# 1879615351/Go-RIO

Hardware: AMD Instinct MI355X
Metric: APD-GICP GN iters/sec on 16k-pt scans + GP-preint windows/sec (higher is better)
Workload: dtype f32 search / f64 accumulate; 1 GPU; C4: 64 scan pairs 16384x16384 + 64 GP windows 1 s @ 200 Hz per GPU, k-NN covariances + 20 fixed GN iterations per pair; pairs_per_gpu=64, target_points=16384, optimizer=GN (convergence test disabled), search=pruned, parallelism=batch shard x1 (no collective)

## Files before the change

go-rio_amd/csrc/ugpm_api.hip:

```cpp
#include <hip/hip_runtime.h>

#include <algorithm>
#include <cstdlib>
#include <chrono>
#include <cstdio>
#include <cstring>
#include <limits>
#include <memory>
#include <string>
#include <atomic>
#include <vector>

#include "../../include/gorio_ugpm.h"
#include "dev_buffer.h"
#include "ugpm_kernels.hip"
#include "ugpm_lpm_out.hip"
#include "ugpm_chunks.h"
#include "ugpm_windows.h"

using namespace gorio;
using namespace gorio::windows;

namespace {

// ... 334 lines not shown
  if (which == 2) {
    if (npad <= 256) ug::ata_kernel<4, 16, kAtaTilesCorr><<<grid, 512, lds(16), sq>>>(r.wins, which, r.nw, ng, decide, dense);
    else if (npad <= 512) ug::ata_kernel<8, 16, kAtaTilesCorr><<<grid, 512, lds(16), sq>>>(r.wins, which, r.nw, ng, decide, dense);
    else ug::ata_kernel<16, 8, kAtaTilesCorr><<<grid, 512, lds(8), sq>>>(r.wins, which, r.nw, ng, decide, dense);
  } else {
    if (npad <= 256) ug::ata_kernel<4, 16, kAtaTilesLm><<<grid, 512, lds(16), sq>>>(r.wins, which, r.nw, ng, decide, dense);
    else ug::ata_kernel<8, 16, kAtaTilesLm><<<grid, 512, lds(16), sq>>>(r.wins, which, r.nw, ng, decide, dense);
  }
}

int enqueue_tables_and_correlation(Ctx& c, Batch& b) {
  const int max_S = b.max_S;
  for (const Run& r : b.runs) {
    {
      Stage st(c, 0, r.s);
      ug::lpm_rot_kernel<<<dim3(r.nw, 5), 320, 0, r.s>>>(r.wins);
      ug::lpm_init_kernel<<<r.nw, 320, 0, r.s>>>(r.wins);
    }
    {
      Stage st(c, 1, r.s);
      ug::gram_kernel<<<dim3(6, r.nw), 256, 0, r.s>>>(r.wins);
      ug::cross_kernel<<<dim3(12, r.nw, (std::max(b.max_G, b.max_V) + ug::kCrossRows - 1) / ug::kCrossRows), 256, sizeof(double) * ug::kCrossRows * (((max_S + 31) / 32) * 32 + 4), r.s>>>(r.wins);
    }
    UHIP(hipEventRecord(r.ev_tab, r.s));
    UHIP(hipStreamWaitEvent(r.s2, r.ev_tab, 0));
    {
      Stage st(c, 2, r.s2);
      ug::corr_jac_kernel<<<dim3(ug::kCorrJacParts, r.nw), 256, 0, r.s2>>>(r.wins);
      UHIP(hipEventRecord(r.ev_jac, r.s2));
      launch_ata(c, max_S, r, 2);
      ug::corr_factor_kernel<<<r.nw, 512, 0, r.s2>>>(r.wins);
// ... 82 lines not shown
    const Run& r = b.runs[g];
    if (problem == 0) {
      UHIP(hipStreamWaitEvent(r.s, r.ev_jac, 0));
      ug::lm_turn_kernel<<<r.nw, 256, 0, r.s>>>(r.wins, c.d_diag + 4 * (size_t)r.g0);
    }
    st_lm[g].reset();
  }
  return 0;
}

int enqueue_finish_and_infer(Ctx& c, Batch& b) {
  for (const Run& r : b.runs) {
    UHIP(hipStreamWaitEvent(r.s, r.ev_corr, 0));
    {
      Stage st(c, 4, r.s);
      ug::finish_kernel<<<r.nw, 256, 0, r.s>>>(r.wins, c.d_diag + 4 * (size_t)r.g0);
      ug::infer_kernel<<<dim3(std::max(1, b.max_infer), r.nw), 256, sizeof(double) * 17 * (6 * b.max_S + 16), r.s>>>(r.wins);
    }
    UHIP(hipEventRecord(r.ev_done, r.s));
  }
  for (size_t g = 1; g < b.runs.size(); ++g) UHIP(hipStreamWaitEvent(c.main.s, b.runs[g].ev_done, 0));
  UHIP(hipGetLastError());
  return 0;
}

int collect(Ctx& c, Batch& b, gorio_ugpm_meas* out, gorio_ugpm_diag* diag, std::vector<int>& unfinished) {
  double* const rec = static_cast<double*>(c.pin_out.get());
  double* const dg = rec + b.total_out;
  int* const fin = reinterpret_cast<int*>(dg + 4 * (size_t)b.nw);
  UHIP(hipMemcpyAsync(fin, c.d_ints, sizeof(int) * kWinInts * (size_t)b.nw, hipMemcpyDeviceToHost, c.main.s));
  UHIP(hipMemcpyAsync(dg, c.d_diag, sizeof(double) * 4 * (size_t)b.nw, hipMemcpyDeviceToHost, c.main.s));
// ... 119 lines not shown
  w->min_freq = 500;
  w->quantum = -1;
  w->state_freq = 50.0;
  w->correlate = 1;
  w->overlap = 8;
  w->vel_bias_std = 0.3;
  w->gyr_bias_std = 0.03;
}

const char* gorio_ugpm_last_error(void) { return g_err.c_str(); }

void gorio_ugpm_debug_set_schedule(int speculative_rot) { g_speculative_rot.store(speculative_rot ? 1 : 0); }

void gorio_ugpm_debug_set_path(int flags) { g_debug_path.store(flags); }

int gorio_ugpm_get_stage_times(double seconds[8], int counts[8]) {
  for (int i = 0; i < 8; ++i) {
    if (seconds) seconds[i] = g_stage_s[i];
    if (counts) counts[i] = g_stage_n[i];
  }
  return 0;
}

int gorio_ugpm_preint_batch(const gorio_ugpm_window* windows, int n_windows, gorio_ugpm_meas* out, gorio_ugpm_diag* diag, int device) {
  if (!windows || n_windows <= 0 || !out) return ufail(GORIO_UGPM_ERR_INVALID, "gorio_ugpm_preint_batch: bad arguments");
  bool any_chunked = false;
  for (int i = 0; i < n_windows; ++i) any_chunked = any_chunked || windows[i].quantum >= 0;
  if (!any_chunked) return preint_batch_flat(windows, n_windows, out, diag, device, false);
  struct Req { int first = 0, count = 0, status = 0; chunks::Plan plan; size_t out0 = 0; };
  std::vector<Req> reqs(n_windows);
// ... 105 lines not shown
```

go-rio_amd/csrc/ugpm_kernels.hip:

```cpp
#include <hip/hip_runtime.h>
#include <math.h>

#include "ugpm_device.h"

namespace gorio {
namespace ug {

__device__ __forceinline__ UgpmWin load_win(const UgpmWin* __restrict__ wins, int i) {
  UgpmWin w;
  __builtin_memcpy(&w, (const __attribute__((address_space(4))) void*)(wins + i), sizeof(UgpmWin));
  return w;
}


#ifndef GORIO_UGPM_XCD
#define GORIO_UGPM_XCD 1
#endif
struct WinPart {
  int win, part, z;
};
__device__ __forceinline__ WinPart xcd_win_part() {
  WinPart r{(int)blockIdx.y, (int)blockIdx.x, (int)blockIdx.z};
#if GORIO_UGPM_XCD
  if (gridDim.y >= 16u && (gridDim.y & 7u) == 0u) {
    const unsigned int inner = gridDim.x * gridDim.z;
    const unsigned int L = blockIdx.x + gridDim.x * (blockIdx.y + gridDim.y * blockIdx.z);
    const unsigned int slot = L >> 3, in = slot % inner;
    r.win = (int)((slot / inner) * 8u + (L & 7u));
    r.part = (int)(in % gridDim.x);
    r.z = (int)(in / gridDim.x);
  }
#endif
  return r;
}

constexpr double kDt = 0.01;
constexpr double kBw = 0.0001;
constexpr double kExpTol = 1e-14;
constexpr double kPi = 3.14159265358979323846;

struct V3 {
  double x, y, z;
};
struct M3 {
  double m[9];
};
__device__ __forceinline__ V3 v3(double x, double y, double z) { return V3{x, y, z}; }
__device__ __forceinline__ V3 operator+(V3 a, V3 b) { return V3{a.x + b.x, a.y + b.y, a.z + b.z}; }
__device__ __forceinline__ V3 operator-(V3 a, V3 b) { return V3{a.x - b.x, a.y - b.y, a.z - b.z}; }
__device__ __forceinline__ V3 operator*(double s, V3 a) { return V3{s * a.x, s * a.y, s * a.z}; }
__device__ __forceinline__ double vnorm(V3 a) { return sqrt(a.x * a.x + a.y * a.y + a.z * a.z); }
__device__ __forceinline__ V3 cross(V3 a, V3 b) { return V3{a.y * b.z - a.z * b.y, a.z * b.x - a.x * b.z, a.x * b.y - a.y * b.x}; }
__device__ __forceinline__ M3 eye3() { return M3{{1, 0, 0, 0, 1, 0, 0, 0, 1}}; }
__device__ __forceinline__ M3 mmul(const M3& a, const M3& b) {
// ... 222 lines not shown
    if (bl == 0) storeM(Rq + (size_t)idx * 9, R);
    else if (bl == 1) storeM(Rq + (size_t)(S + idx) * 9, R);
    else if (bl == 2) storeM(w.Rstart + variant * 9, R);
    else if (bl == 4 && variant == 0) {
      const V3 vr = mvec(R, v3(w.vel[idx] - w.vel_bias[0], w.vel[V + idx] - w.vel_bias[1], w.vel[2 * V + idx] - w.vel_bias[2]));
      w.velr[idx] = vr.x;
      w.velr[V + idx] = vr.y;
      w.velr[2 * V + idx] = vr.z;
    }
    interp(bt, w_prev);
    t_prev = bt;
  }
}

constexpr int kLpmMaxT = 2048;
struct LpmLds {
  double tl[kLpmMaxT];
  unsigned short kind[kLpmMaxT];
  unsigned short kidx[kLpmMaxT];
  double tot[2][256][9];
  double ps[9];
  int start_rank;
};

__device__ __forceinline__ int lower_bound_f(int n, double v, const double* __restrict__ a, double shift) {
  int lo = 0, hi = n;
  while (lo < hi) {
    const int mid = (lo + hi) >> 1;
    if (a[mid] - shift < v) lo = mid + 1; else hi = mid;
  }
  return lo;
}
__device__ __forceinline__ int upper_bound_f(int n, double v, const double* __restrict__ a, double shift) {
  int lo = 0, hi = n;
  while (lo < hi) {
    const int mid = (lo + hi) >> 1;
    if (a[mid] - shift <= v) lo = mid + 1; else hi = mid;
  }
  return lo;
}

__device__ bool lpm_rotation_parallel(const UgpmWin& w, int variant, LpmLds& L, double* __restrict__ Rseq , size_t rseq_cap) {
  const int S = w.S, G = w.G, V = w.V;
  const int nthr = blockDim.x, tid = threadIdx.x;
  const double lpm_start = w.state_t[0];
  const double tshift = variant == 1 ? kDt : 0.0;
  int nfake = 0;
  double fake_first = 0.0, fake_q = 0.0;
  {
    double first = w.state_t[0], top1 = -1e300, top2 = -1e300;
    auto consider = [&](double c) {
      if (c > top1) { top2 = top1; top1 = c; } else if (c > top2) { top2 = c; }
    };
    consider(w.state_t[S - 1]); if (S > 1) consider(w.state_t[S - 2]);
    consider(w.state_t[S - 1] + kDt); if (S > 1) consider(w.state_t[S - 2] + kDt);
    consider(w.start_t);
    consider(lpm_start + kDt); consider(lpm_start);
    consider(w.vel_t[V - 1] - tshift); if (V > 1) consider(w.vel_t[V - 2] - tshift);
    first = fmin(first, fmin(w.start_t, w.vel_t[0] - tshift));
    if ((top1 - top2) > (1.0 / 500.0)) {
      const int nb = (int)floor((top1 - first) * 500.0);
      if (nb > 0) { nfake = nb; fake_first = first; fake_q = (top1 - first) / ((double)nb); }
    }
  }
  const int T = 2 * S + 3 + V + nfake;
  if (T > kLpmMaxT || (size_t)T * 9 > rseq_cap) return false;
  auto count_in = [&](int l, double v, bool upper) -> int {
    switch (l) {
      case 0: return upper ? upper_bound_f(S, v, w.state_t, 0.0) : lower_bound_f(S, v, w.state_t, 0.0);
      case 1: return upper ? upper_bound_f(S, v, w.state_t, -kDt) : lower_bound_f(S, v, w.state_t, -kDt);
      case 2: return upper ? (w.start_t <= v ? 1 : 0) : (w.start_t < v ? 1 : 0);
      case 3: { const double a0 = lpm_start, a1 = lpm_start + kDt; return upper ? ((a0 <= v) + (a1 <= v)) : ((a0 < v) + (a1 < v)); }
      case 4: return upper ? upper_bound_f(V, v, w.vel_t, tshift) : lower_bound_f(V, v, w.vel_t, tshift);
      default: {
        int lo = 0, hi = nfake;
        while (lo < hi) {
          const int mid = (lo + hi) >> 1;
          const double c = fake_first + mid * fake_q;
          if (upper ? (c <= v) : (c < v)) lo = mid + 1; else hi = mid;
        }
        return lo;
      }
    }
  };
  const int prio[6] = {1, 2, 3, 0, 4, 5};
  const int nl[6] = {S, S, 1, 2, V, nfake};
  for (int e = tid; e < T; e += nthr) {
    int l = 0, i = e;
    while (i >= nl[l]) { i -= nl[l]; ++l; }
    double v;
    switch (l) {
      case 0: v = w.state_t[i]; break;
      case 1: v = w.state_t[i] + kDt; break;
      case 2: v = w.start_t; break;
      case 3: v = lpm_start + (i ? kDt : 0.0); break;
      case 4: v = w.vel_t[i] - tshift; break;
      default: v = fake_first + i * fake_q; break;
    }
    int rank = i;
    for (int b = 0; b < 6; ++b)
      if (b != l && nl[b] > 0) rank += count_in(b, v, prio[b] < prio[l]);
    L.tl[rank] = v;
    L.kind[rank] = (unsigned short)l;
    L.kidx[rank] = (unsigned short)i;
    if (l == 3 && i == 0) L.start_rank = rank;
  }
  __syncthreads();
  auto gt = [&](int i) -> double { return w.gyr_t[i] - tshift; };
  auto gd = [&](int a, int i) -> double {
    double d = w.gyr[a * G + i];
    if (variant == 0) d -= w.gyr_bias[a];
    if (variant - 2 == a) d += kBw;
    return d;
  };
  const double gt0 = gt(0);
  auto step_rot = [&](int i) -> M3 {
    const double t = L.tl[i];
    int p = 0;
    if (t > gt0) {
      p = lower_bound_f(G, t, w.gyr_t, tshift) - 1;
      if (p > G - 2) p = G - 2;
      if (p < 0) p = 0;
    }
    const double t0 = gt(p), t1 = gt(p + 1);
    double wv[3];
    for (int a = 0; a < 3; ++a) {
      const double d0 = gd(a, p), d1 = gd(a, p + 1);
      const double al = (d1 - d0) / (t1 - t0);
      const double be = d0 - (al * t0);
      wv[a] = al * t + be;
    }
    const double dt = L.tl[i + 1] - t;
    return expMap(v3(wv[0] * dt, wv[1] * dt, wv[2] * dt));
  };
  const int nch = nthr < 256 ? nthr : 256;
  const int ch = (T + nch - 1) / nch;
  if (tid < nch) {
    M3 acc = eye3();
    const int i0 = tid * ch, i1 = min(T, i0 + ch);
    for (int i = i0; i < i1; ++i) {
      storeM(Rseq + (size_t)i * 9, acc);
      if (i < T - 1) acc = mmul(acc, step_rot(i));
    }
    storeM(&L.tot[0][tid][0], acc);
  }
  __syncthreads();
  int cur = 0;
  for (int off = 1; off < nch; off <<= 1) {
    if (tid < nch) {
      M3 m = loadM(&L.tot[cur][tid][0]);
      if (tid >= off) m = mmul(loadM(&L.tot[cur][tid - off][0]), m);
      storeM(&L.tot[cur ^ 1][tid][0], m);
    }
    __syncthreads();
    cur ^= 1;
  }
  if (tid < nch) {
    const M3 pre = tid > 0 ? loadM(&L.tot[cur][tid - 1][0]) : eye3();
    const int i0 = tid * ch, i1 = min(T, i0 + ch);
    for (int i = i0; i < i1; ++i) {
      const M3 Pi = mmul(pre, loadM(Rseq + (size_t)i * 9));
      storeM(Rseq + (size_t)i * 9, Pi);
      if (i == L.start_rank) storeM(L.ps, mtr(Pi));
    }
  }
  __syncthreads();
  const M3 PsT = loadM(L.ps);
  double* Rq = w.Rq + (size_t)variant * 2 * S * 9;
  for (int i = tid; i < T; i += nthr) {
    const int l = L.kind[i], idx = L.kidx[i];
    if (l == 5 || l == 3) continue;
    if (l == 4 && variant != 0) continue;
    const M3 Pi = loadM(Rseq + (size_t)i * 9);
    const M3 R = i >= L.start_rank ? mmul(PsT, Pi) : Pi;
    if (l == 0) storeM(Rq + (size_t)idx * 9, R);
    else if (l == 1) storeM(Rq + (size_t)(S + idx) * 9, R);
    else if (l == 2) storeM(w.Rstart + variant * 9, R);
    else {
      const V3 vr = mvec(R, v3(w.vel[idx] - w.vel_bias[0], w.vel[V + idx] - w.vel_bias[1], w.vel[2 * V + idx] - w.vel_bias[2]));
      w.velr[idx] = vr.x;
      w.velr[V + idx] = vr.y;
      w.velr[2 * V + idx] = vr.z;
    }
  }
  __syncthreads();
  return true;
}

__device__ void lpm_position(const UgpmWin& w, int axis) {
  const int S = w.S, V = w.V;
  const double start = w.state_t[0];
  const double* vt = w.vel_t;
  const double* vd = w.velr + (size_t)axis * V;
  int data_ptr = 0;
  while (vt[data_ptr + 1] < start) {
    data_ptr++;
    if (data_ptr == V - 1) {
      *w.status = -3;
      return;
    }
// ... 60 lines not shown
          if (d < best) {
            best = d;
            id = q;
            bc = c;
          }
        }
        prev[j] = bc;
        rev[j] += (id - 1);
      }
      store3(r0 + (size_t)i * 3, prev[0]);
      store3(r1 + (size_t)i * 3, prev[1]);
    }
  }
}

__global__ __launch_bounds__(320) void lpm_rot_kernel(const UgpmWin* __restrict__ wins) {
  const UgpmWin w = load_win(wins, blockIdx.x);
  if (*w.status != 0) return;
  const int var = blockIdx.y, lane = threadIdx.x & 63;
  __shared__ LpmLds lds;
  {
    const size_t cap = ((size_t)(3 * w.S + 3 * w.G) * 3 * w.S) / 5;
    double* Rseq = w.Jrot + (size_t)var * cap;
    if (!lpm_rotation_parallel(w, var, lds, Rseq, cap)) {
      if (threadIdx.x == 0) lpm_rotation(w, var);
    }
  }
  __syncthreads();
  if (var == 0 && threadIdx.x < 3) lpm_position(w, threadIdx.x);
  if (threadIdx.x == 64) unwrap_variant(w, var);
  (void)lane;
}

__device__ void lm_begin_block(const UgpmWin& w, int problem);

__global__ __launch_bounds__(320) void lpm_init_kernel(const UgpmWin* __restrict__ wins) {
  const UgpmWin w = load_win(wins, blockIdx.x);
  if (*w.status != 0) return;
  const int S = w.S;
  const M3 sRt0 = mtr(loadM(w.Rstart));
  for (int i = threadIdx.x; i < S; i += blockDim.x) {
    const V3 a0 = load3(w.r0 + (size_t)i * 3), a1 = load3(w.r1 + (size_t)i * 3);
    const V3 d = (1.0 / kDt) * (a1 - a0);
    w.s_dr[i] = d.x; w.s_dr[S + i] = d.y; w.s_dr[2 * S + i] = d.z;
    const V3 vel = mvec(sRt0, (1.0 / kDt) * (load3(w.dp + ((size_t)S + i) * 3) - load3(w.dp + (size_t)i * 3)));
    w.s_vel[i] = vel.x; w.s_vel[S + i] = vel.y; w.s_vel[2 * S + i] = vel.z;
// ... 1427 lines not shown
  {
    const int rows = ((n + 15) / 16 - jb) * 16;
    for (int q = threadIdx.x; q < rows * 16; q += blockDim.x) Xc[(size_t)(q >> 4) * 17 + (q & 15)] = (q >> 4) == (q & 15) ? 1.0 : 0.0;
  }
  blocked_lower_solve16(w.Ac, n, jb, Xc, sh);
  if (threadIdx.x < 16) {
    const int c = threadIdx.x, col = j0 + c;
    const int rows = ((n + 15) / 16 - jb) * 16;
    double ssq = 0.0;
    for (int r = 0; r < rows; ++r) ssq = __builtin_fma(Xc[(size_t)r * 17 + c], Xc[(size_t)r * 17 + c], ssq);
    if (col < n) w.dsc[col] = w.sstd[col] * (1.0 / sqrt(ssq));
  }
}


__global__ __launch_bounds__(256) void finish_kernel(const UgpmWin* __restrict__ wins, double* __restrict__ diag_out ) {
  const UgpmWin w = load_win(wins, blockIdx.x);
  if (*w.status != 0) return;
  if (!lm_end_block(w, 1, diag_out + 4 * (size_t)blockIdx.x)) return;
  __syncthreads();
  const int S = w.S;
  for (int q = threadIdx.x; q < 6 * S; q += blockDim.x) {
    const int c = q / S, i = q % S;
    const double* s = c < 3 ? w.s_dr + (size_t)c * S : w.s_vel + (size_t)(c - 3) * S;
    w.alpha[q] = row_dot(w.Kinv + ((size_t)c * S + i) * S, s, S);
  }
  for (int q = threadIdx.x; q < 3 * S; q += blockDim.x) {
    const int a = q / S, i = q % S;
    w.state_r[q] = row_dot(w.KintKinv + ((size_t)a * S + i) * S, w.s_dr + (size_t)a * S, S) + (w.state_t[i] - w.start_t) * w.hyper[a * 4 + 3];
  }
  __syncthreads();
  for (int i = threadIdx.x; i < S; i += blockDim.x) {
    const V3 ri = v3(w.state_r[i], w.state_r[S + i], w.state_r[2 * S + i]);
    const M3 Ji = JrInv(ri);
    const V3 d_r = mvec(Ji, load3(w.d_r_dt_local + (size_t)i * 3));
// ... 32 lines not shown
      }
    const V3 sv = v3(w.s_vel[i], w.s_vel[S + i], w.s_vel[2 * S + i]) + mean_vel;
    const M3 dvbw = mmul(mmul(skew(sv), Jr(v3(-ri.x, -ri.y, -ri.z))), drbw);
    const V3 dvdt = (1.0 / kDt) * (mvec(dRt, sv) - sv);
    const double dv[3] = {dvdt.x, dvdt.y, dvdt.z};
    for (int a = 0; a < 3; ++a) {
      for (int c = 0; c < 3; ++c) {
        w.d_vel_bv[((size_t)a * S + i) * 3 + c] = R.m[a * 3 + c];
        w.d_vel_bw[((size_t)a * S + i) * 3 + c] = -dvbw.m[a * 3 + c];
      }
      w.d_vel_dt[a * S + i] = dv[a];
    }
  }
}

__global__ __launch_bounds__(256) void infer_kernel(const UgpmWin* __restrict__ wins) {
  const WinPart wp = xcd_win_part();
  const UgpmWin w = load_win(wins, wp.win);
  const int qi = wp.part;
  if (qi >= w.n_infer) return;
  double* out = w.out + (size_t)qi * 83;
  if (*w.status != 0) {
    for (int k = threadIdx.x; k < 83; k += blockDim.x) out[k] = __longlong_as_double(0x7ff8000000000000LL);
    return;
  }
  const int S = w.S, n = 6 * S;
  const double t = w.infer_t[qi], dt = t - w.start_t;
  __shared__ double ksv[6][160];
  __shared__ double ksd[3][160];
  __shared__ double ksK[6][160];
  __shared__ double sval[6][8];
  __shared__ double sval2[6][4];
  __shared__ double sred[8];
  __shared__ double scov[36];
  for (int q = threadIdx.x; q < 6 * S; q += blockDim.x) {
    const int c = q / S, j = q - c * S;
    ksv[c][j] = se_kint(w.start_t, t, w.state_t[j], w.hyper[c * 4], w.hyper[c * 4 + 1]);
    if (c >= 3) ksd[c - 3][j] = se_kint_dt(w.start_t, t, w.state_t[j], w.hyper[c * 4], w.hyper[c * 4 + 1]);
  }
  __syncthreads();
  for (int q = threadIdx.x; q < 6 * S; q += blockDim.x) {
    const int c = q / S, j = q - c * S;
    const double* Kc = w.Kinv + (size_t)c * S * S + j;
    double s = 0.0;
    for (int k = 0; k < S; ++k) s += ksv[c][k] * Kc[(size_t)k * S];
    ksK[c][j] = s;
  }
  __syncthreads();
  {
    const int wv = threadIdx.x >> 6, lane = threadIdx.x & 63;
    for (int c = wv; c < 6; c += (int)(blockDim.x >> 6)) {
      double acc[9] = {0, 0, 0, 0, 0, 0, 0, 0, 0};
      for (int j = lane; j < S; j += 64) {
        const double ks = ksv[c][j], kk = ksK[c][j];
        acc[0] += ks * w.alpha[c * S + j];
        acc[1] += kk * ks;
        if (c < 3) {
          acc[2] += kk * w.d_d_r_dt[c * S + j];
          for (int q = 0; q < 3; ++q) acc[3 + q] += kk * w.d_state_bw[((size_t)c * S + j) * 3 + q];
        } else {
          acc[2] += ksd[c - 3][j] * w.alpha[c * S + j] + kk * w.d_vel_dt[(c - 3) * S + j];
          for (int q = 0; q < 3; ++q) {
            acc[3 + q] += kk * w.d_vel_bw[((size_t)(c - 3) * S + j) * 3 + q];
// ... 8 lines not shown
      if (lane == 0) {
        const double l2 = w.hyper[c * 4], sf2 = w.hyper[c * 4 + 1];
        double var = kss_int(w.start_t, t, l2, sf2) - acc[1];
        if (var <= 0) var = dt * dt * w.hyper[c * 4 + 2];
        sval[c][0] = acc[0] + dt * w.hyper[c * 4 + 3];
        sval[c][1] = var;
        sval[c][2] = acc[2];
        for (int q = 0; q < 3; ++q) {
          sval[c][3 + q] = acc[3 + q];
          sval2[c][q] = acc[6 + q];
        }
      }
    }
  }
  __syncthreads();
  if (w.correlate) {
    extern __shared__ double Xc[];
    __shared__ Solve16Lds sh;
    const int rows = ((n + 15) / 16) * 16;
    for (int q = threadIdx.x; q < rows * 16; q += blockDim.x) Xc[(size_t)(q >> 4) * 17 + (q & 15)] = 0.0;
    __syncthreads();
    for (int row = threadIdx.x; row < n; row += blockDim.x) {
      const int c = row / S;
      Xc[(size_t)row * 17 + c] = w.dsc[row] * ksK[c][row - c * S];
    }
    blocked_lower_solve16(w.Ac, n, 0, Xc, sh);
    for (int pair = 0; pair < 21; ++pair) {
      int a2 = 0, b2 = pair;
      while (b2 >= 6 - a2) { b2 -= 6 - a2; ++a2; }
      b2 += a2;
      double acc = 0.0;
      for (int k = threadIdx.x; k < rows; k += blockDim.x) acc += Xc[(size_t)k * 17 + a2] * Xc[(size_t)k * 17 + b2];
      acc = block_sum(acc, sred);
      if (threadIdx.x == 0) {
        scov[a2 * 6 + b2] = acc;
        scov[b2 * 6 + a2] = acc;
      }
    }
  } else {
    if (threadIdx.x < 36) scov[threadIdx.x] = 0.0;
    __syncthreads();
    if (threadIdx.x < 6) {
      const int a2 = threadIdx.x;
      double s2 = 0.0;
      for (int j = 0; j < S; ++j) s2 += ksK[a2][j] * w.var[a2 * S + j] * ksK[a2][j];
      scov[a2 * 6 + a2] = s2;
    }
  }
  __syncthreads();
  if (threadIdx.x == 0) {
    const V3 r = v3(sval[0][0], sval[1][0], sval[2][0]);
    const M3 jr = Jr(r);
    const M3 R = expMap(r);
    M3 d_r_dw, d_p_dw, d_p_dv;
    for (int a = 0; a < 3; ++a)
      for (int q = 0; q < 3; ++q) {
        d_r_dw.m[a * 3 + q] = sval[a][3 + q];
        d_p_dw.m[a * 3 + q] = sval[3 + a][3 + q];
        d_p_dv.m[a * 3 + q] = sval2[3 + a][q];
      }
    storeM(out, R);
    out[9] = sval[3][0]; out[10] = sval[4][0]; out[11] = sval[5][0];
    out[12] = dt;
    out[13] = 0.5 * dt * dt;
// ... 28 lines not shown
      }
      for (int a = 0; a < 6; ++a)
        for (int b = 0; b < 6; ++b) {
          double s = 0.0;
          for (int k = 0; k < 6; ++k) s += J[a * 6 + k] * bc[k] * J[b * 6 + k];
          cov[a * 6 + b] += s;
        }
    }
    for (int q = 0; q < 36; ++q) out[14 + q] = cov[q];
    storeM(out + 50, mmul(jr, d_r_dw));
    store3(out + 59, mvec(jr, v3(sval[0][2], sval[1][2], sval[2][2])));
    storeM(out + 62, d_p_dw);
    storeM(out + 71, d_p_dv);
    out[80] = sval[3][2]; out[81] = sval[4][2]; out[82] = sval[5][2];
  }
}

}
}
```

go-rio_amd/ugpm.py:

```python
import ctypes as C

import numpy as np

from .apd import GorioError, load_library

LPM, UGPM = 0, 1
REC = 83

UGPM_SYMBOLS = ["gorio_ugpm_default_window", "gorio_ugpm_preint_batch", "gorio_ugpm_last_error", "gorio_ugpm_get_stage_times", "gorio_ugpm_debug_set_schedule",
                "gorio_ugpm_debug_set_path",                 "gorio_ugpm_combine_preints"]


class UgpmWindow(C.Structure):

    _fields_ = [
        ("gyr_t", C.c_void_p), ("gyr", C.c_void_p), ("n_gyr", C.c_int),
        ("vel_t", C.c_void_p), ("vel", C.c_void_p), ("n_vel", C.c_int),
        ("gyr_var", C.c_double), ("vel_var", C.c_double), ("start_t", C.c_double),
        ("infer_t", C.c_void_p), ("n_infer", C.c_int), ("type", C.c_int),
        ("min_freq", C.c_double), ("quantum", C.c_double), ("state_freq", C.c_double),
        ("correlate", C.c_int), ("overlap", C.c_int),
        ("gyr_bias", C.c_double * 3), ("vel_bias", C.c_double * 3),
        ("vel_bias_std", C.c_double), ("gyr_bias_std", C.c_double),
        ("group_sizes", C.c_void_p), ("n_groups", C.c_int),
# ... 98 lines not shown
    a, b, out = np.ascontiguousarray(pack(prev)), np.ascontiguousarray(pack(cur)), np.zeros(REC)
    lib.gorio_ugpm_combine_preints.argtypes = [C.c_void_p, C.c_void_p, C.c_void_p]
    rc = lib.gorio_ugpm_combine_preints(C.c_void_p(_dp(a)), C.c_void_p(_dp(b)), C.c_void_p(_dp(out)))
    if rc < 0:
        raise GorioError(rc, lib.gorio_ugpm_last_error().decode())
    return unpack(out)


def ugpm_debug_set_schedule(speculative_rot=True):
    lib = load_library()
    lib.gorio_ugpm_debug_set_schedule.argtypes = [C.c_int]
    lib.gorio_ugpm_debug_set_schedule.restype = None
    lib.gorio_ugpm_debug_set_schedule(1 if speculative_rot else 0)


def ugpm_debug_set_path(dense_ata=False, draining_looks=False):
    lib = load_library()
    lib.gorio_ugpm_debug_set_path.argtypes = [C.c_int]
    lib.gorio_ugpm_debug_set_path.restype = None
    lib.gorio_ugpm_debug_set_path((1 if dense_ata else 0) | (2 if draining_looks else 0))


def ugpm_stage_times():
    lib = load_library()
    s = (C.c_double * 8)()
    c = (C.c_int * 8)()
    lib.gorio_ugpm_get_stage_times(s, c)
    return list(s), list(c)


class PreintOption:

    def __init__(self, min_freq=500.0, type=UGPM, quantum=-1.0, state_freq=50.0, correlate=True):
        self.min_freq, self.type, self.quantum, self.state_freq, self.correlate = min_freq, type, quantum, state_freq, correlate

# ... 59 lines not shown
```

Baseline: 180,800 linearisations/s.

## Parallelise UGPM head/tail stages: staged LDS timestamps, parallel position/unwrap, tiled finish dots

Stages the state, velocity and gyro timestamp arrays into LDS for the LPM rotation kernel and packs the kind/index arrays into one word. The formerly single-thread position integration and unwrap tail are replaced by a parallel precompute of segment coefficients, query ranks and log maps, leaving only a short serial sweep. finish_kernel now computes its row dot products through LDS-tiled loads, and infer_kernel's 21 covariance reductions are fused into a single pass with wave shuffles. A debug flag keeps the old serial path, and optional cycle-counter instrumentation is added behind a compile macro.

```diff
diff --git a/go-rio_amd/csrc/ugpm_api.hip b/go-rio_amd/csrc/ugpm_api.hip
--- a/go-rio_amd/csrc/ugpm_api.hip
+++ b/go-rio_amd/csrc/ugpm_api.hip
@@ -372,7 +372,7 @@
   for (const Run& r : b.runs) {
     {
       Stage st(c, 0, r.s);
-      ug::lpm_rot_kernel<<<dim3(r.nw, 5), 320, 0, r.s>>>(r.wins);
+      ug::lpm_rot_kernel<<<dim3(r.nw, 5), 320, 0, r.s>>>(r.wins, (g_debug_path.load() & 4) ? 1 : 0);
       ug::lpm_init_kernel<<<r.nw, 320, 0, r.s>>>(r.wins);
     }
     {
@@ -485,7 +485,7 @@
     UHIP(hipStreamWaitEvent(r.s, r.ev_corr, 0));
     {
       Stage st(c, 4, r.s);
-      ug::finish_kernel<<<r.nw, 256, 0, r.s>>>(r.wins, c.d_diag + 4 * (size_t)r.g0);
+      ug::finish_kernel<<<r.nw, 256, 0, r.s>>>(r.wins, c.d_diag + 4 * (size_t)r.g0, (g_debug_path.load() & 4) ? 1 : 0);
       ug::infer_kernel<<<dim3(std::max(1, b.max_infer), r.nw), 256, sizeof(double) * 17 * (6 * b.max_S + 16), r.s>>>(r.wins);
     }
     UHIP(hipEventRecord(r.ev_done, r.s));
@@ -635,6 +635,15 @@
 
 void gorio_ugpm_debug_set_path(int flags) { g_debug_path.store(flags); }
 
+#ifdef GORIO_HT_TIMING
+int gorio_ugpm_debug_head_tail_cycles(long long cycles[32]) {
+  long long z[32] = {};
+  if (hipDeviceSynchronize() != hipSuccess) return -1;
+  if (cycles && hipMemcpyFromSymbol(cycles, HIP_SYMBOL(gorio::ug::g_ht_t), sizeof z) != hipSuccess) return -1;
+  return hipMemcpyToSymbol(HIP_SYMBOL(gorio::ug::g_ht_t), z, sizeof z) == hipSuccess ? 0 : -1;
+}
+#endif
+
 int gorio_ugpm_get_stage_times(double seconds[8], int counts[8]) {
   for (int i = 0; i < 8; ++i) {
     if (seconds) seconds[i] = g_stage_s[i];
diff --git a/go-rio_amd/csrc/ugpm_kernels.hip b/go-rio_amd/csrc/ugpm_kernels.hip
--- a/go-rio_amd/csrc/ugpm_kernels.hip
+++ b/go-rio_amd/csrc/ugpm_kernels.hip
@@ -38,6 +38,24 @@
 constexpr double kBw = 0.0001;
 constexpr double kExpTol = 1e-14;
 constexpr double kPi = 3.14159265358979323846;
+
+#ifdef GORIO_HT_TIMING
+__device__ long long g_ht_t[32];
+#define HT_T(k, thr)                                                                        \
+  do {                                                                                      \
+    if (blockIdx.x == 0 && blockIdx.y == 0 && (int)threadIdx.x == (thr)) {                  \
+      const long long now_ = (long long)__builtin_readcyclecounter();                       \
+      g_ht_t[k] += now_ - ht_last_;                                                         \
+      ht_last_ = now_;                                                                      \
+    }                                                                                       \
+  } while (0)
+#define HT_T_INIT long long ht_last_ = (long long)__builtin_readcyclecounter()
+#define HT_T_RESET ht_last_ = (long long)__builtin_readcyclecounter()
+#else
+#define HT_T(k, thr) do { } while (0)
+#define HT_T_INIT do { } while (0)
+#define HT_T_RESET do { } while (0)
+#endif
 
 struct V3 {
   double x, y, z;
@@ -290,14 +308,26 @@
 }
 
 constexpr int kLpmMaxT = 2048;
+constexpr int kLpmStage = 1000;
+constexpr int kLpmPos = 2 * 256 * 9;
 struct LpmLds {
-  double tl[kLpmMaxT];
-  unsigned short kind[kLpmMaxT];
-  unsigned short kidx[kLpmMaxT];
-  double tot[2][256][9];
+  union {
+    struct {
+      double tl[kLpmMaxT];
+      unsigned short kk[kLpmMaxT];
+    } line;
+    double uw[2 * 160 * 7];
+  };
+  union {
+    double tot[2][256][9];
+    double pos[kLpmPos];
+  };
+  double stage[kLpmStage];
   double ps[9];
   int start_rank;
+  int data_ptr;
 };
+static_assert(sizeof(LpmLds) <= 65536, "lpm_rot_kernel: static LDS");
 
 __device__ __forceinline__ int lower_bound_f(int n, double v, const double* __restrict__ a, double shift) {
   int lo = 0, hi = n;
@@ -316,24 +346,29 @@
   return lo;
 }
 
-__device__ bool lpm_rotation_parallel(const UgpmWin& w, int variant, LpmLds& L, double* __restrict__ Rseq , size_t rseq_cap) {
+template <bool STAGED>
+__device__ __forceinline__ bool lpm_rotation_parallel(const UgpmWin& w, int variant, LpmLds& L, double* __restrict__ Rseq , size_t rseq_cap) {
   const int S = w.S, G = w.G, V = w.V;
   const int nthr = blockDim.x, tid = threadIdx.x;
-  const double lpm_start = w.state_t[0];
+  const double* __restrict__ st = STAGED ? L.stage : w.state_t;
+  const double* __restrict__ vt = STAGED ? L.stage + S : w.vel_t;
+  const double* __restrict__ gl = STAGED ? L.stage + S + V : w.gyr_t;
+  const double lpm_start = st[0];
   const double tshift = variant == 1 ? kDt : 0.0;
+  HT_T_INIT;
   int nfake = 0;
   double fake_first = 0.0, fake_q = 0.0;
   {
-    double first = w.state_t[0], top1 = -1e300, top2 = -1e300;
+    double first = st[0], top1 = -1e300, top2 = -1e300;
     auto consider = [&](double c) {
       if (c > top1) { top2 = top1; top1 = c; } else if (c > top2) { top2 = c; }
     };
-    consider(w.state_t[S - 1]); if (S > 1) consider(w.state_t[S - 2]);
-    consider(w.state_t[S - 1] + kDt); if (S > 1) consider(w.state_t[S - 2] + kDt);
+    consider(st[S - 1]); if (S > 1) consider(st[S - 2]);
+    consider(st[S - 1] + kDt); if (S > 1) consider(st[S - 2] + kDt);
     consider(w.start_t);
     consider(lpm_start + kDt); consider(lpm_start);
-    consider(w.vel_t[V - 1] - tshift); if (V > 1) consider(w.vel_t[V - 2] - tshift);
-    first = fmin(first, fmin(w.start_t, w.vel_t[0] - tshift));
+    consider(vt[V - 1] - tshift); if (V > 1) consider(vt[V - 2] - tshift);
+    first = fmin(first, fmin(w.start_t, vt[0] - tshift));
     if ((top1 - top2) > (1.0 / 500.0)) {
       const int nb = (int)floor((top1 - first) * 500.0);
       if (nb > 0) { nfake = nb; fake_first = first; fake_q = (top1 - first) / ((double)nb); }
@@ -343,11 +378,11 @@
   if (T > kLpmMaxT || (size_t)T * 9 > rseq_cap) return false;
   auto count_in = [&](int l, double v, bool upper) -> int {
     switch (l) {
-      case 0: return upper ? upper_bound_f(S, v, w.state_t, 0.0) : lower_bound_f(S, v, w.state_t, 0.0);
-      case 1: return upper ? upper_bound_f(S, v, w.state_t, -kDt) : lower_bound_f(S, v, w.state_t, -kDt);
+      case 0: return upper ? upper_bound_f(S, v, st, 0.0) : lower_bound_f(S, v, st, 0.0);
+      case 1: return upper ? upper_bound_f(S, v, st, -kDt) : lower_bound_f(S, v, st, -kDt);
       case 2: return upper ? (w.start_t <= v ? 1 : 0) : (w.start_t < v ? 1 : 0);
       case 3: { const double a0 = lpm_start, a1 = lpm_start + kDt; return upper ? ((a0 <= v) + (a1 <= v)) : ((a0 < v) + (a1 < v)); }
-      case 4: return upper ? upper_bound_f(V, v, w.vel_t, tshift) : lower_bound_f(V, v, w.vel_t, tshift);
+      case 4: return upper ? upper_bound_f(V, v, vt, tshift) : lower_bound_f(V, v, vt, tshift);
       default: {
         int lo = 0, hi = nfake;
         while (lo < hi) {
@@ -366,23 +401,23 @@
     while (i >= nl[l]) { i -= nl[l]; ++l; }
     double v;
     switch (l) {
-      case 0: v = w.state_t[i]; break;
-      case 1: v = w.state_t[i] + kDt; break;
+      case 0: v = st[i]; break;
+      case 1: v = st[i] + kDt; break;
       case 2: v = w.start_t; break;
       case 3: v = lpm_start + (i ? kDt : 0.0); break;
-      case 4: v = w.vel_t[i] - tshift; break;
+      case 4: v = vt[i] - tshift; break;
       default: v = fake_first + i * fake_q; break;
     }
     int rank = i;
     for (int b = 0; b < 6; ++b)
       if (b != l && nl[b] > 0) rank += count_in(b, v, prio[b] < prio[l]);
-    L.tl[rank] = v;
-    L.kind[rank] = (unsigned short)l;
-    L.kidx[rank] = (unsigned short)i;
+    L.line.tl[rank] = v;
+    L.line.kk[rank] = (unsigned short)(l << 11 | i);
     if (l == 3 && i == 0) L.start_rank = rank;
   }
   __syncthreads();
-  auto gt = [&](int i) -> double { return w.gyr_t[i] - tshift; };
+  HT_T(0, 0);
+  auto gt = [&](int i) -> double { return gl[i] - tshift; };
   auto gd = [&](int a, int i) -> double {
     double d = w.gyr[a * G + i];
     if (variant == 0) d -= w.gyr_bias[a];
@@ -391,10 +426,10 @@
   };
   const double gt0 = gt(0);
   auto step_rot = [&](int i) -> M3 {
-    const double t = L.tl[i];
+    const double t = L.line.tl[i];
     int p = 0;
     if (t > gt0) {
-      p = lower_bound_f(G, t, w.gyr_t, tshift) - 1;
+      p = lower_bound_f(G, t, gl, tshift) - 1;
       if (p > G - 2) p = G - 2;
       if (p < 0) p = 0;
     }
@@ -406,7 +441,7 @@
       const double be = d0 - (al * t0);
       wv[a] = al * t + be;
     }
-    const double dt = L.tl[i + 1] - t;
+    const double dt = L.line.tl[i + 1] - t;
     return expMap(v3(wv[0] * dt, wv[1] * dt, wv[2] * dt));
   };
   const int nch = nthr < 256 ? nthr : 256;
@@ -421,6 +456,7 @@
     storeM(&L.tot[0][tid][0], acc);
   }
   __syncthreads();
+  HT_T(1, 0);
   int cur = 0;
   for (int off = 1; off < nch; off <<= 1) {
     if (tid < nch) {
@@ -431,6 +467,7 @@
     __syncthreads();
     cur ^= 1;
   }
+  HT_T(2, 0);
   if (tid < nch) {
     const M3 pre = tid > 0 ? loadM(&L.tot[cur][tid - 1][0]) : eye3();
     const int i0 = tid * ch, i1 = min(T, i0 + ch);
@@ -441,10 +478,11 @@
     }
   }
   __syncthreads();
+  HT_T(3, 0);
   const M3 PsT = loadM(L.ps);
   double* Rq = w.Rq + (size_t)variant * 2 * S * 9;
   for (int i = tid; i < T; i += nthr) {
-    const int l = L.kind[i], idx = L.kidx[i];
+    const int l = L.line.kk[i] >> 11, idx = L.line.kk[i] & 2047;
     if (l == 5 || l == 3) continue;
     if (l == 4 && variant != 0) continue;
     const M3 Pi = loadM(Rseq + (size_t)i * 9);
@@ -460,6 +498,7 @@
     }
   }
   __syncthreads();
+  HT_T(4, 0);
   return true;
 }
 
@@ -550,22 +589,179 @@
   }
 }
 
-__global__ __launch_bounds__(320) void lpm_rot_kernel(const UgpmWin* __restrict__ wins) {
+__device__ __forceinline__ void lpm_tail_parallel(const UgpmWin& w, int var, LpmLds& L, bool staged) {
+  HT_T_INIT;
+  const int S = w.S, V = w.V, NQ = 2 * S + 1;
+  const int nthr = blockDim.x, tid = threadIdx.x;
+  const bool postab = var == 0 && staged && 12 * V + 2 * NQ <= kLpmPos;
+  const double* __restrict__ st = L.stage;
+  const double* __restrict__ vt = L.stage + S;
+  double* __restrict__ al = L.pos;
+  double* __restrict__ be = al + 3 * V;
+  double* __restrict__ ar = be + 3 * V;
+  double* __restrict__ d0 = ar + 3 * V;
+  double* __restrict__ qt = d0 + 3 * V;
+  int* __restrict__ qk = (int*)(qt + NQ);
+  const double start = w.state_t[0];
+  {
+    const M3 sRt = mtr(loadM(w.Rstart + var * 9));
+    const double* Rq = w.Rq + (size_t)var * 2 * S * 9;
+    for (int e = tid; e < 2 * S; e += nthr) {
+      const V3 tr = logMap(mmul(sRt, loadM(Rq + (size_t)e * 9)));
+      const double nr = vnorm(tr);
+      V3 u = tr;
+      if (nr != 0) u = (1.0 / nr) * tr;
+      double* o = L.uw + e * 7;
+      store3(o, tr);
+      o[3] = nr;
+      store3(o + 4, u);
+    }
+  }
+  if (postab) {
+    for (int p = tid; p < V - 1; p += nthr)
+      if (!(vt[p + 1] < start)) {
+        atomicMin(&L.data_ptr, p);
+        break;
+      }
+    for (int e = tid; e < NQ; e += nthr) {
+      const int l = e < S ? 0 : (e < 2 * S ? 1 : 2), i = e - l * S;
+      int rank;
+      double v;
+      if (l == 0) {
+        v = st[i];
+        rank = i + lower_bound_f(S, v, st, -kDt) + (w.start_t < v ? 1 : 0);
+      } else if (l == 1) {
+        v = st[i] + kDt;
+        rank = i + upper_bound_f(S, v, st, 0.0) + (w.start_t < v ? 1 : 0);
+      } else {
+        v = w.start_t;
+        rank = upper_bound_f(S, v, st, 0.0) + upper_bound_f(S, v, st, -kDt);
+      }
+      qt[rank] = v;
+      qk[rank] = l < 2 ? e : -1;
+    }
+  }
+  __syncthreads();
+  HT_T(20, 0);
+  const int dp0 = L.data_ptr;
+  if (postab && dp0 < V - 1) {
+    const int nseg = V - 1 - dp0;
+    for (int q = tid; q < 3 * nseg; q += nthr) {
+      const int axis = q / nseg, p = dp0 + (q - axis * nseg);
+      const double* vd = w.velr + (size_t)axis * V;
+      const double t_lo = vt[p], t_1 = vt[p + 1], d_lo = vd[p], d_1 = vd[p + 1];
+      const double alpha = (d_1 - d_lo) / (t_1 - t_lo);
+      const double beta = d_lo - alpha * t_lo;
+      const double t_0 = p == dp0 ? start : t_lo;
+      const double d_0 = p == dp0 ? alpha * t_lo + beta : d_lo;
+      al[axis * V + p] = alpha;
+      be[axis * V + p] = beta;
+      d0[axis * V + p] = d_0;
+      ar[axis * V + p] = (t_1 - t_0) * (d_0 + d_1) / 2.0;
+    }
+  }
+  __syncthreads();
+  HT_T(21, 0);
+  if (var == 0 && tid < 3) {
+    if (!postab) {
+      lpm_position(w, tid);
+    } else if (dp0 >= V - 1) {
+      if (tid == 0) *w.status = -3;
+    } else {
+      const int axis = tid;
+      const double vt0 = vt[0];
+      int ptr = dp0;
+      double backup = 0.0, lo = vt[ptr], hi = vt[ptr + 1];
+      for (int step = 0; step < NQ; ++step) {
+        const double t = qt[step];
+        const int k = qk[step];
+        if (t > vt0) {
+          while (true) {
+            if ((t >= lo) && (t <= hi)) break;
+            if (ptr < (V - 2)) {
+              backup = backup + ar[axis * V + ptr];
+              ptr++;
+              lo = hi;
+              hi = vt[ptr + 1];
+            } else {
+              break;
+            }
+          }
+        }
+        const double t_0 = ptr == dp0 ? start : lo;
+        const double temp_d_1 = al[axis * V + ptr] * t + be[axis * V + ptr];
+        const double temp_d_p = backup + ((t - t_0) * (d0[axis * V + ptr] + temp_d_1) / 2.0);
+        if (k >= 0 && k < 2 * S) w.dp[(size_t)k * 3 + axis] = temp_d_p;
+      }
+    }
+  }
+  HT_T(5, 0);
+  if (tid >= 64 && tid < 68) {
+    const int j = (tid - 64) & 1, pass = (tid - 64) >> 1;
+    const int from = pass == 0 ? w.overlap : w.overlap - 1, cnt = pass == 0 ? S - w.overlap : w.overlap, stp = pass == 0 ? 1 : -1;
+    double* rj = (j == 0 ? w.r0 : w.r1) + (size_t)var * S * 3;
+    int rev = 0;
+    V3 prev = v3(0, 0, 0);
+    for (int n = 0; n < cnt; ++n) {
+      const int i = from + n * stp;
+      const double* o = L.uw + (j * S + i) * 7;
+      const V3 tr = load3(o), u = load3(o + 4);
+      const double nr = o[3];
+      int id = 0;
+      double best = 1.7976931348623157e308;
+      V3 bc = tr;
+      for (int q = 0; q < 3; ++q) {
+        const int m = rev + q - 1;
+        V3 c = tr;
+        if (nr != 0) c = (2.0 * kPi * m + nr) * u;
+        const double d = vnorm(prev - c);
+        if (d < best) {
+          best = d;
+          id = q;
+          bc = c;
+        }
+      }
+      prev = bc;
+      rev += (id - 1);
+      store3(rj + (size_t)i * 3, prev);
+    }
+  }
+  HT_T(6, 64);
+}
+
+__global__ __launch_bounds__(320) void lpm_rot_kernel(const UgpmWin* __restrict__ wins, int serial) {
   const UgpmWin w = load_win(wins, blockIdx.x);
   if (*w.status != 0) return;
-  const int var = blockIdx.y, lane = threadIdx.x & 63;
+  const int var = blockIdx.y;
   __shared__ LpmLds lds;
+  HT_T_INIT;
+  const bool staged = !serial && w.S + w.V + w.G <= kLpmStage;
+  if (staged) {
+    for (int i = threadIdx.x; i < w.S; i += blockDim.x) lds.stage[i] = w.state_t[i];
+    for (int i = threadIdx.x; i < w.V; i += blockDim.x) lds.stage[w.S + i] = w.vel_t[i];
+    for (int i = threadIdx.x; i < w.G; i += blockDim.x) lds.stage[w.S + w.V + i] = w.gyr_t[i];
+  }
+  if (threadIdx.x == 0) lds.data_ptr = w.V - 1;
+  __syncthreads();
+  HT_T(7, 0);
   {
     const size_t cap = ((size_t)(3 * w.S + 3 * w.G) * 3 * w.S) / 5;
     double* Rseq = w.Jrot + (size_t)var * cap;
-    if (!lpm_rotation_parallel(w, var, lds, Rseq, cap)) {
+    const bool fits = staged ? lpm_rotation_parallel<true>(w, var, lds, Rseq, cap) : lpm_rotation_parallel<false>(w, var, lds, Rseq, cap);
+    if (!fits) {
       if (threadIdx.x == 0) lpm_rotation(w, var);
     }
   }
   __syncthreads();
-  if (var == 0 && threadIdx.x < 3) lpm_position(w, threadIdx.x);
-  if (threadIdx.x == 64) unwrap_variant(w, var);
-  (void)lane;
+  HT_T_RESET;
+  if (serial) {
+    if (var == 0 && threadIdx.x < 3) lpm_position(w, threadIdx.x);
+    HT_T(5, 0);
+    if (threadIdx.x == 64) unwrap_variant(w, var);
+    HT_T(6, 64);
+    return;
+  }
+  lpm_tail_parallel(w, var, lds, staged);
 }
 
 __device__ void lm_begin_block(const UgpmWin& w, int problem);
@@ -2023,11 +2219,46 @@
 }
 
 
-__global__ __launch_bounds__(256) void finish_kernel(const UgpmWin* __restrict__ wins, double* __restrict__ diag_out ) {
-  const UgpmWin w = load_win(wins, blockIdx.x);
-  if (*w.status != 0) return;
-  if (!lm_end_block(w, 1, diag_out + 4 * (size_t)blockIdx.x)) return;
-  __syncthreads();
+constexpr int kDotTile = 4608;
+template <int NC, class F>
+__device__ __forceinline__ void tiled_row_dots(const double* __restrict__ M, int nrows, int S, double* __restrict__ tile, F&& f) {
+  const int ld = S | 1;
+  const int tr = min(kDotTile / ld, (int)blockDim.x / NC);
+  for (int r0 = 0; r0 < nrows; r0 += tr) {
+    const int nr = min(tr, nrows - r0);
+    __syncthreads();
+    {
+      const double* __restrict__ src = M + (size_t)r0 * S;
+      const int n = nr * S, dr = (int)blockDim.x / S, dc = (int)blockDim.x - dr * S;
+      int r = (int)threadIdx.x / S, c = (int)threadIdx.x - r * S;
+      for (int q0 = threadIdx.x; q0 < n; q0 += 8 * blockDim.x) {
+        double v[8];
+#pragma unroll
+        for (int u = 0; u < 8; ++u) {
+          const int q = q0 + u * (int)blockDim.x;
+          v[u] = q < n ? src[q] : 0.0;
+        }
+#pragma unroll
+        for (int u = 0; u < 8; ++u) {
+          if (q0 + u * (int)blockDim.x < n) tile[r * ld + c] = v[u];
+          r += dr;
+          c += dc;
+          if (c >= S) {
+            c -= S;
+            ++r;
+          }
+        }
+      }
+    }
+    __syncthreads();
+    if ((int)threadIdx.x < nr * NC) {
+      const int r = threadIdx.x / NC;
+      f(r0 + r, (int)threadIdx.x - r * NC, tile + r * ld);
+    }
+  }
+}
+
+__device__ void finish_serial(const UgpmWin& w) {
   const int S = w.S;
   for (int q = threadIdx.x; q < 6 * S; q += blockDim.x) {
     const int c = q / S, i = q % S;
@@ -2090,6 +2321,93 @@
   }
 }
 
+__global__ __launch_bounds__(256) void finish_kernel(const UgpmWin* __restrict__ wins, double* __restrict__ diag_out , int serial) {
+  const UgpmWin w = load_win(wins, blockIdx.x);
+  if (*w.status != 0) return;
+  HT_T_INIT;
+  if (!lm_end_block(w, 1, diag_out + 4 * (size_t)blockIdx.x)) return;
+  __syncthreads();
+  HT_T(8, 0);
+  if (serial) {
+    finish_serial(w);
+    return;
+  }
+  const int S = w.S;
+  __shared__ double tile[kDotTile];
+  __shared__ double vec[9 * 160];
+  __shared__ double sums[9 * 160];
+  __shared__ double srd[3];
+  for (int q = threadIdx.x; q < 6 * S; q += blockDim.x) vec[q] = q < 3 * S ? w.s_dr[q] : w.s_vel[q - 3 * S];
+  tiled_row_dots<1>(w.Kinv, 6 * S, S, tile, [&](int q, int, const double* row) {
+    w.alpha[q] = row_dot(row, vec + (q / S) * S, S);
+  });
+  tiled_row_dots<1>(w.KintKinv, 3 * S, S, tile, [&](int q, int, const double* row) {
+    const int a = q / S, i = q % S;
+    w.state_r[q] = row_dot(row, vec + a * S, S) + (w.state_t[i] - w.start_t) * w.hyper[a * 4 + 3];
+  });
+  __syncthreads();
+  HT_T(9, 0);
+  for (int i = threadIdx.x; i < S; i += blockDim.x) {
+    const V3 ri = v3(w.state_r[i], w.state_r[S + i], w.state_r[2 * S + i]);
+    const M3 Ji = JrInv(ri);
+    const V3 d_r = mvec(Ji, load3(w.d_r_dt_local + (size_t)i * 3));
+    const V3 temp_r = ri + mvec(Ji, load3(w.delta_r_time + (size_t)i * 3));
+    const V3 dd = (1.0 / kDt) * (mvec(JrInv(temp_r), load3(w.d_r_dt_local_shift + (size_t)i * 3)) - d_r);
+    w.d_d_r_dt[i] = dd.x; w.d_d_r_dt[S + i] = dd.y; w.d_d_r_dt[2 * S + i] = dd.z;
+    for (int ax = 0; ax < 3; ++ax) {
+      const V3 trw = ri + mvec(Ji, load3(w.delta_r_bw + ((size_t)ax * S + i) * 3));
+      const V3 t = (1.0 / kBw) * (mvec(JrInv(trw), load3(w.d_r_bw_local_shift + ((size_t)ax * S + i) * 3)) - d_r);
+      for (int a = 0; a < 3; ++a) {
+        const double ta = a == 0 ? t.x : (a == 1 ? t.y : t.z);
+        w.d_state_bw[((size_t)a * S + i) * 3 + ax] = ta;
+        vec[(a * S + i) * 3 + ax] = ta;
+      }
+    }
+  }
+  for (int q = threadIdx.x; q < 3 * S; q += blockDim.x) {
+    const int c = q / S, j = q - c * S;
+    tile[q] = se_kint(w.start_t, w.start_t + kDt, w.state_t[j], w.hyper[c * 4], w.hyper[c * 4 + 1]) * w.alpha[q];
+  }
+  __syncthreads();
+  HT_T(10, 0);
+  if (threadIdx.x < 3) {
+    const int c = threadIdx.x;
+    double s = 0.0;
+    for (int j = 0; j < S; ++j) s += tile[c * S + j];
+    srd[c] = s + kDt * w.hyper[c * 4 + 3];
+  }
+  __syncthreads();
+  HT_T(11, 0);
+  tiled_row_dots<3>(w.KintKinv, 3 * S, S, tile, [&](int q, int c, const double* row) {
+    const int a = q / S;
+    double s = 0.0;
+    for (int j = 0; j < S; ++j) s += row[j] * vec[(a * S + j) * 3 + c];
+    sums[q * 3 + c] = s;
+  });
+  __syncthreads();
+  const M3 dRt = mtr(expMap(v3(srd[0], srd[1], srd[2])));
+  const V3 mean_vel = v3(w.hyper[15], w.hyper[19], w.hyper[23]);
+  for (int i = threadIdx.x; i < S; i += blockDim.x) {
+    const V3 ri = v3(w.state_r[i], w.state_r[S + i], w.state_r[2 * S + i]);
+    const M3 R = expMap(ri);
+    M3 drbw;
+    for (int a = 0; a < 3; ++a)
+      for (int c = 0; c < 3; ++c) drbw.m[a * 3 + c] = sums[(a * S + i) * 3 + c];
+    const V3 sv = v3(w.s_vel[i], w.s_vel[S + i], w.s_vel[2 * S + i]) + mean_vel;
+    const M3 dvbw = mmul(mmul(skew(sv), Jr(v3(-ri.x, -ri.y, -ri.z))), drbw);
+    const V3 dvdt = (1.0 / kDt) * (mvec(dRt, sv) - sv);
+    const double dv[3] = {dvdt.x, dvdt.y, dvdt.z};
+    for (int a = 0; a < 3; ++a) {
+      for (int c = 0; c < 3; ++c) {
+        w.d_vel_bv[((size_t)a * S + i) * 3 + c] = R.m[a * 3 + c];
+        w.d_vel_bw[((size_t)a * S + i) * 3 + c] = -dvbw.m[a * 3 + c];
+      }
+      w.d_vel_dt[a * S + i] = dv[a];
+    }
+  }
+  HT_T(12, 0);
+}
+
 __global__ __launch_bounds__(256) void infer_kernel(const UgpmWin* __restrict__ wins) {
   const WinPart wp = xcd_win_part();
   const UgpmWin w = load_win(wins, wp.win);
@@ -2109,12 +2427,14 @@
   __shared__ double sval2[6][4];
   __shared__ double sred[8];
   __shared__ double scov[36];
+  HT_T_INIT;
   for (int q = threadIdx.x; q < 6 * S; q += blockDim.x) {
     const int c = q / S, j = q - c * S;
     ksv[c][j] = se_kint(w.start_t, t, w.state_t[j], w.hyper[c * 4], w.hyper[c * 4 + 1]);
     if (c >= 3) ksd[c - 3][j] = se_kint_dt(w.start_t, t, w.state_t[j], w.hyper[c * 4], w.hyper[c * 4 + 1]);
   }
   __syncthreads();
+  HT_T(14, 0);
   for (int q = threadIdx.x; q < 6 * S; q += blockDim.x) {
     const int c = q / S, j = q - c * S;
     const double* Kc = w.Kinv + (size_t)c * S * S + j;
@@ -2123,6 +2443,7 @@
     ksK[c][j] = s;
   }
   __syncthreads();
+  HT_T(15, 0);
   {
     const int wv = threadIdx.x >> 6, lane = threadIdx.x & 63;
     for (int c = wv; c < 6; c += (int)(blockDim.x >> 6)) {
@@ -2161,6 +2482,7 @@
     }
   }
   __syncthreads();
+  HT_T(16, 0);
   if (w.correlate) {
     extern __shared__ double Xc[];
     __shared__ Solve16Lds sh;
@@ -2172,16 +2494,37 @@
       Xc[(size_t)row * 17 + c] = w.dsc[row] * ksK[c][row - c * S];
     }
     blocked_lower_solve16(w.Ac, n, 0, Xc, sh);
-    for (int pair = 0; pair < 21; ++pair) {
-      int a2 = 0, b2 = pair;
-      while (b2 >= 6 - a2) { b2 -= 6 - a2; ++a2; }
-      b2 += a2;
-      double acc = 0.0;
-      for (int k = threadIdx.x; k < rows; k += blockDim.x) acc += Xc[(size_t)k * 17 + a2] * Xc[(size_t)k * 17 + b2];
-      acc = block_sum(acc, sred);
-      if (threadIdx.x == 0) {
-        scov[a2 * 6 + b2] = acc;
-        scov[b2 * 6 + a2] = acc;
+    HT_T(17, 0);
+    {
+      double(*sred21)[4] = reinterpret_cast<double(*)[4]>(&sh.Pt[0][0][0]);
+      double acc[21];
+#pragma unroll
+      for (int pair = 0; pair < 21; ++pair) acc[pair] = 0.0;
+      for (int k = threadIdx.x; k < rows; k += blockDim.x) {
+        double x[6];
+#pragma unroll
+        for (int c = 0; c < 6; ++c) x[c] = Xc[(size_t)k * 17 + c];
+        int pair = 0;
+#pragma unroll
+        for (int a2 = 0; a2 < 6; ++a2)
+#pragma unroll
+          for (int b2 = a2; b2 < 6; ++b2) acc[pair++] += x[a2] * x[b2];
+      }
+#pragma unroll
+      for (int pair = 0; pair < 21; ++pair) {
+#pragma unroll
+        for (int off = 32; off > 0; off >>= 1) acc[pair] += __shfl_down(acc[pair], off, 64);
+        if ((threadIdx.x & 63) == 0) sred21[pair][threadIdx.x >> 6] = acc[pair];
+      }
+      __syncthreads();
+      if (threadIdx.x < 21) {
+        int a2 = 0, b2 = threadIdx.x;
+        while (b2 >= 6 - a2) { b2 -= 6 - a2; ++a2; }
+        b2 += a2;
+        double t = 0.0;
+        for (int q = 0; q < (int)(blockDim.x >> 6); ++q) t += sred21[threadIdx.x][q];
+        scov[a2 * 6 + b2] = t;
+        scov[b2 * 6 + a2] = t;
       }
     }
   } else {
@@ -2195,6 +2538,7 @@
     }
   }
   __syncthreads();
+  HT_T(18, 0);
   if (threadIdx.x == 0) {
     const V3 r = v3(sval[0][0], sval[1][0], sval[2][0]);
     const M3 jr = Jr(r);
@@ -2253,7 +2597,8 @@
     storeM(out + 71, d_p_dv);
     out[80] = sval[3][2]; out[81] = sval[4][2]; out[82] = sval[5][2];
   }
-}
-
-}
-}
+  HT_T(19, 0);
+}
+
+}
+}
diff --git a/go-rio_amd/ugpm.py b/go-rio_amd/ugpm.py
--- a/go-rio_amd/ugpm.py
+++ b/go-rio_amd/ugpm.py
@@ -136,11 +136,11 @@
     lib.gorio_ugpm_debug_set_schedule(1 if speculative_rot else 0)
 
 
-def ugpm_debug_set_path(dense_ata=False, draining_looks=False):
+def ugpm_debug_set_path(dense_ata=False, draining_looks=False, serial_head_tail=False):
     lib = load_library()
     lib.gorio_ugpm_debug_set_path.argtypes = [C.c_int]
     lib.gorio_ugpm_debug_set_path.restype = None
-    lib.gorio_ugpm_debug_set_path((1 if dense_ata else 0) | (2 if draining_looks else 0))
+    lib.gorio_ugpm_debug_set_path((1 if dense_ata else 0) | (2 if draining_looks else 0) | (4 if serial_head_tail else 0))
 
 
 def ugpm_stage_times():
```

Measured after the change: 178,800 linearisations/s. 1.1% lower.
